# saiprasadbarke/robustmvd

Measured on AMD Instinct MI355X. Metric: depth-maps/sec at 768x1152x4srcx256planes; warp+aggregate HBM GB/s vs roofline, higher is better.
Workload: dtype f32; 1 GPU; mvsnet (Path B) forward 768x1152, 4 source views, 256 planes, batch 1 per step (BASELINE.json configs[2]); the regulariser's two layers with 32 input channels (conv0, conv4): every fp32 operand as two range-scaled fp16 terms on fp16 MFMA, fp32 accumulation (at least as close to a float64 convolution as the fp32 matrix instruction over 1e-42..1e30: tests/test_hip_f16.py), the other nine layers and ; parallelism=1 independent replica(s), frames round-robin, no collectives

## Files before the change

### robustmvd_amd/csrc/conv3d.hip

```cpp
#include "mvd_common.h"
#include <stdlib.h>

namespace mvd {

typedef float f32x4 __attribute__((ext_vector_type(4)));
typedef float f32x2 __attribute__((ext_vector_type(2)));
typedef unsigned int u32x4c __attribute__((ext_vector_type(4)));

constexpr int CONV_TH = 4;
constexpr int CONV_PAD = 4;

struct ConvParams {
    const float* x;
    const float* wpk;
    const float* scale;
    const float* shift;
    const float* skip;
    float* y;
    float* absmax;
    int B, Di, hi, wi;
    int Do, ho, wo;
    int Cout;
    int relu;
    int tiles_w, tiles_h;
    int per_xcd;
};

__device__ __forceinline__ int tile_index(const ConvParams& p) {
    const int bx = blockIdx.x;
    return (p.per_xcd > 0 && bx < 8 * p.per_xcd) ? (bx % 8) * p.per_xcd + bx / 8 : bx;
}
static int xcd_run(long long nblk, int bit) {
    const char* e = exp_env("MVD_K4_XCD");
    return (e && ((atoi(e) >> bit) & 1)) ? (int)(nblk / 8) : 0;
}

template <int CIN>
struct KGroup {
    static constexpr int KG = CIN >= 16 ? 16 : CIN;
    static constexpr int R = KG / 4;
    static constexpr int NKG = CIN / KG;
};

template <int CIN>
__host__ __device__ constexpr size_t packed_floats(int nt, int taps = 27) {
    return (size_t)taps * KGroup<CIN>::NKG * nt * 64 * KGroup<CIN>::R;
}
constexpr int MVD_CONV3D_S1_PAIR = 3;


template <int R>
__device__ __forceinline__ void load_frag(const float* src, float (&dst)[R]) {
    static_assert(R == 4 || R == 2, "k-groups of 16 or 8 channels");
    if constexpr (R == 4) {
        const float4 t = *reinterpret_cast<const float4*>(src);
        dst[0] = t.x; dst[1] = t.y; dst[2] = t.z; dst[3] = t.w;
    } else {
        const float2 t = *reinterpret_cast<const float2*>(src);
        dst[0] = t.x; dst[1] = t.y;
    }
}

__device__ __forceinline__ int decode_tile(const ConvParams& p, int bx, int& tw, int& th) {
    tw = bx % p.tiles_w; bx /= p.tiles_w;
    th = bx % p.tiles_h;
    return bx / p.tiles_h;
}

template <int CIN>
__global__ void pack_weights_kernel(const float* __restrict__ w, float* __restrict__ packed, int Cout, int NT,
                                    int transposed) {
    using G = KGroup<CIN>;
    const bool pair = transposed == 2;
    const bool dpair = transposed == 3;
    const size_t total = packed_floats<CIN>(NT, pair ? 36 : dpair ? 18 : 27);
    for (size_t e = (size_t)blockIdx.x * blockDim.x + threadIdx.x; e < total; e += (size_t)gridDim.x * blockDim.x) {
        size_t r = e;
        const int j = r % G::R; r /= G::R;
        const int lane = r % 64; r /= 64;
        const int nt = r % NT; r /= NT;
        const int g = r % G::NKG; r /= G::NKG;
        const int tap = (int)r;
        const int row = nt * 16 + (lane & 15);
        const int cin = g * G::KG + G::R * (lane >> 4) + j;
        float val = 0.f;
        if (pair) {
            const int phase = row >> 3, cout = row & 7;
            const int t = tap & 3, kdh = tap >> 2;
            const int kw = t - phase;
            if (kw >= 0 && kw <= 2) val = w[((size_t)cout * CIN + cin) * 27 + kdh * 3 + kw];
        } else if (dpair) {
            const int pw = row >> 3, cout = row & 7;
            const int st = tap & 1, kdh = tap >> 1;
            const int kw = st == 0 ? (pw ? 2 : 1) : (pw ? 0 : -1);
            if (kw >= 0) val = w[((size_t)cin * 8 + cout) * 27 + kdh * 3 + kw];
        } else if (row < Cout) {
            val = transposed ? w[((size_t)cin * Cout + row) * 27 + tap]
                             : w[((size_t)row * CIN + cin) * 27 + tap];
        }
        packed[e] = val;
    }
}

template <int MODE, int MT>
struct TileGeom {
    static constexpr bool S2 = MODE == MVD_CONV3D_STRIDE2, DECONV = MODE == MVD_DECONV3D_STRIDE2, PAIR = MODE == MVD_CONV3D_S1_PAIR;
    static constexpr int TW = 16 * MT;
    static constexpr int SX = (S2 || PAIR) ? 2 : 1;
// ... 902 lines not shown
                    for (int m = 0; m < MT; ++m)
                        acc[cls][m] = __builtin_amdgcn_mfma_f32_16x16x4f32(af[st][g][j], bf[m][j], acc[cls][m], 0, 0, 0);
            }
        }
        if (kdh + 1 < 9) {
#pragma unroll
            for (int st = 0; st < 2; ++st)
#pragma unroll
                for (int g = 0; g < G::NKG; ++g)
#pragma unroll
                    for (int j = 0; j < G::R; ++j) af[st][g][j] = af_next[st][g][j];
        }
    }

    const int arow = r0 + wave;
    if (arow >= p.hi) return;
    constexpr unsigned OOB = 0x80000000u;
    unsigned coff[MT];
#pragma unroll
    for (int m = 0; m < MT; ++m) {
        const int gcol = c0 + m * 16 + vox;
        coff[m] = gcol < p.wi ? (unsigned)(((size_t)2 * gcol * 8 + q * 4) * 4) : OOB;
    }
    const int row_bytes = p.wo * 8 * 4;
    float4 sk[4][MT];
    __amdgpu_buffer_rsrc_t yrs[4];
#pragma unroll
    for (int c = 0; c < 4; ++c) {
        const int pd = c >> 1, ph = c & 1;
        const size_t row_base = (((size_t)b * p.Do + 2 * zd + pd) * p.ho + 2 * arow + ph) * p.wo * 8;
        yrs[c] = __builtin_amdgcn_make_buffer_rsrc(p.y + row_base, 0, row_bytes, 0x00020000);
        const __amdgpu_buffer_rsrc_t srs = __builtin_amdgcn_make_buffer_rsrc(
            const_cast<float*>(p.skip ? p.skip + row_base : p.y), 0, p.skip ? row_bytes : 0, 0x00020000);
#pragma unroll
        for (int m = 0; m < MT; ++m) {
            const u32x4c t = __builtin_amdgcn_raw_buffer_load_b128(srs, coff[m], 0, 0);
            sk[c][m] = make_float4(__uint_as_float(t[0]), __uint_as_float(t[1]), __uint_as_float(t[2]), __uint_as_float(t[3]));
        }
    }
#pragma unroll
    for (int c = 0; c < 4; ++c)
#pragma unroll
        for (int m = 0; m < MT; ++m) {
            float r[4];
#pragma unroll
            for (int k = 0; k < 4; ++k) {
                r[k] = fmaf(acc[c][m][k], esc[k], esh[k]);
                if (p.relu) r[k] = fmaxf(r[k], 0.f);
            }
            __builtin_amdgcn_raw_buffer_store_b128(u32x4c{__float_as_uint(r[0] + sk[c][m].x), __float_as_uint(r[1] + sk[c][m].y),
                                                          __float_as_uint(r[2] + sk[c][m].z), __float_as_uint(r[3] + sk[c][m].w)},
                                                   yrs[c], coff[m], 0, 0);
        }
}

template <int CIN, int MT>
static int launch_deconv_pair(const ConvParams& p0, hipStream_t st) {
    ConvParams p = p0;
    constexpr size_t lds = (size_t)2 * (CONV_TH + 1) * (16 * MT + 1) * (CIN + CONV_PAD) * sizeof(float);
    static_assert(lds <= 160 * 1024, "slab exceeds LDS");
    p.tiles_h = (p.hi + CONV_TH - 1) / CONV_TH;
    p.tiles_w = (p.wi + 16 * MT - 1) / (16 * MT);
    const long long nblk = (long long)p.tiles_w * p.tiles_h * p.Di * p.B;
    p.per_xcd = xcd_run(nblk, 1);
    return launch_tiles(deconv3d_pair_kernel<CIN, MT>, nblk, 256, lds, "deconv3d_pair", p, st);
}

template <int CIN, int NT, int MT>
static int launch_deconv_all(const ConvParams& p0, hipStream_t st) {
    ConvParams p = p0;
    constexpr size_t lds = (size_t)2 * (CONV_TH + 1) * (16 * MT + 1) * (CIN + CONV_PAD) * sizeof(float);
    static_assert(lds <= 160 * 1024, "slab exceeds LDS");
    p.tiles_h = (p.hi + CONV_TH - 1) / CONV_TH;
    p.tiles_w = (p.wi + 16 * MT - 1) / (16 * MT);
    const long long nblk = (long long)p.tiles_w * p.tiles_h * p.Di * p.B;
    return launch_tiles(deconv3d_all_kernel<CIN, NT, MT>, nblk, 256, lds, "deconv3d_all", p, st);
}

constexpr int C8_DZ = 16;
constexpr int C8_TW = 62;
__global__ void __launch_bounds__(256, 4) conv3d_c8_to_1_kernel(ConvParams p) {
    constexpr int CIN = 8, TW = C8_TW, ROWS = CONV_TH + 2, COLS = TW + 2, PSTR = CIN, SLAB = ROWS * COLS * PSTR;
    static_assert(COLS == 64, "one slab column per lane");
    constexpr int NEL = ROWS * COLS * 2, NPF = (NEL + 255) / 256, DZ = C8_DZ;
    __shared__ __attribute__((aligned(16))) float ring[3 * SLAB + 4];
    const int tid = threadIdx.x, lane = tid & 63, wave = tid >> 6;
    int tw, th;
    const int bx = decode_tile(p, tile_index(p), tw, th);
    const int nzc = (p.Do + DZ - 1) / DZ;
    const int zc = bx % nzc;
    const int b = bx / nzc;
    const int r0 = th * CONV_TH, c0 = tw * TW;
    const int z0 = zc * DZ, z1 = min(z0 + DZ, p.Do);

    int loff[NPF], goff[NPF];
#pragma unroll
    for (int i = 0; i < NPF; ++i) {
        const int e = tid + 256 * i;
        const int row = e / (COLS * 2), rem = e - row * (COLS * 2);
        const int col = rem >> 1, c4 = rem & 1;
        const int gr = r0 - 1 + row, gc = c0 - 1 + col;
        constexpr int DUMMY = (3 * SLAB) / 4;
        loff[i] = e < NEL ? ((row * COLS + col) * PSTR) / 4 + c4 : DUMMY;
        goff[i] = (e < NEL && gr >= 0 && gr < p.hi && gc >= 0 && gc < p.wi) ? (gr * p.wi + gc) * 2 + c4 : -1;
    }
    const size_t plane_f4 = (size_t)p.hi * p.wi * 2;
    const float4* __restrict__ xb = reinterpret_cast<const float4*>(p.x) + (size_t)b * p.Di * plane_f4;
    float4* __restrict__ ring4 = reinterpret_cast<float4*>(ring);
    float4 pf[NPF];
    bool pf_ok = false;
    auto load_plane = [&](int plane) {
        const bool ok = plane >= 0 && plane < p.Di;
        const float4* __restrict__ xp = xb + (size_t)(ok ? plane : 0) * plane_f4;
        pf_ok = ok;
#pragma unroll
        for (int i = 0; i < NPF; ++i) pf[i] = xp[max(goff[i], 0)];
    };
    auto store_plane = [&](int slot) {
        constexpr int DUMMY = (3 * SLAB) / 4;
#pragma unroll
        for (int i = 0; i < NPF; ++i)
            ring4[loff[i] == DUMMY ? DUMMY : slot * (SLAB / 4) + loff[i]] =
                (pf_ok && goff[i] >= 0) ? pf[i] : make_float4(0.f, 0.f, 0.f, 0.f);
    };
    load_plane(z0 - 1);
    store_plane((z0 + 2) % 3);
    load_plane(z0);
    store_plane(z0 % 3);
    load_plane(z0 + 1);

    const int orow = r0 + wave, ocol = c0 + lane - 1;
    const bool live = lane >= 1 && lane <= TW && orow < p.ho && ocol < p.wo;
    const float sc = p.scale[0], sh = p.shift[0];
    for (int z = z0; z < z1; ++z) {
        __syncthreads();
        store_plane((z + 1) % 3);
        __syncthreads();
        if (z + 1 < z1) load_plane(z + 2);
        f32x2 qa[3], qb[3];
#pragma unroll
        for (int kw = 0; kw < 3; ++kw) { qa[kw] = f32x2{0.f, 0.f}; qb[kw] = f32x2{0.f, 0.f}; }
#pragma unroll
        for (int kd = 0; kd < 3; ++kd) {
            const float* __restrict__ slab = ring + ((z + kd + 2) % 3) * SLAB;
#pragma unroll
            for (int kh = 0; kh < 3; ++kh) {
                const f32x4* sp = reinterpret_cast<const f32x4*>(slab + ((wave + kh) * COLS + lane) * PSTR);
                const f32x4 a = sp[0], c = sp[1];
#pragma unroll
                for (int kw = 0; kw < 3; ++kw) {
                    typedef const __attribute__((address_space(4))) f32x4* cf4;
                    const cf4 wp = (cf4)(unsigned long long)(p.wpk + ((kd * 3 + kh) * 3 + kw) * 8);
                    const f32x4 w0 = wp[0], w1 = wp[1];
                    qa[kw] = __builtin_elementwise_fma(a.xy, w0.xy, qa[kw]);
                    qb[kw] = __builtin_elementwise_fma(a.zw, w0.zw, qb[kw]);
                    qa[kw] = __builtin_elementwise_fma(c.xy, w1.xy, qa[kw]);
                    qb[kw] = __builtin_elementwise_fma(c.zw, w1.zw, qb[kw]);
                }
            }
        }
        float q[3];
#pragma unroll
        for (int kw = 0; kw < 3; ++kw) q[kw] = (qa[kw].x + qa[kw].y) + (qb[kw].x + qb[kw].y);
        const float acc = (__shfl_up(q[0], 1) + q[1]) + __shfl_down(q[2], 1);
        if (live) {
            const size_t o = (((size_t)b * p.Do + z) * p.ho + orow) * p.wo + ocol;
            float val = fmaf(acc, sc, sh);
            if (p.relu) val = fmaxf(val, 0.f);
            if (p.skip) val += p.skip[o];
            p.y[o] = val;
        }
    }
}

__global__ void pack_c8_to_1_kernel(const float* __restrict__ w, float* __restrict__ packed) {
    const int e = blockIdx.x * blockDim.x + threadIdx.x;
    if (e < 216) packed[e] = w[(e % 8) * 27 + e / 8];
}

template <int CIN, int NT, int MT, int MODE>
static int launch_conv(const ConvParams& p0, hipStream_t st) {
    ConvParams p = p0;
    using T = TileGeom<MODE, MT>;
    constexpr size_t lds = (size_t)T::ROWS * T::COLS * (CIN + CONV_PAD) * sizeof(float) + 16;
    static_assert(lds <= 160 * 1024, "slab exceeds LDS");
    const int gh = T::DECONV ? p.hi : p.ho;
    const int gw = T::DECONV ? p.wi : T::PAIR ? (p.wo + 1) / 2 : p.wo;
    p.tiles_h = (gh + CONV_TH - 1) / CONV_TH;
    p.tiles_w = (gw + T::TW - 1) / T::TW;
    const long long nz = T::DECONV ? (long long)p.Di * 4 : p.Do;
    const long long nblk = (long long)p.tiles_w * p.tiles_h * nz * p.B;
    return launch_tiles(conv3d_kernel<CIN, NT, MT, MODE>, nblk, 256, lds, "conv3d", p, st);
}

static int launch_c8_to_1(const ConvParams& p0, hipStream_t st) {
    ConvParams p = p0;
    p.tiles_h = (p.ho + CONV_TH - 1) / CONV_TH;
    p.tiles_w = (p.wo + C8_TW - 1) / C8_TW;
    const long long nblk = (long long)p.tiles_w * p.tiles_h * ((p.Do + C8_DZ - 1) / C8_DZ) * p.B;
    p.per_xcd = xcd_run(nblk, 0);
    return launch_tiles(conv3d_c8_to_1_kernel, nblk, 256, 0, "conv3d_c8_to_1", p, st);
}

static int best_mt(int cols, int lo, int hi) {
    int best = hi, waste = 1 << 30;
    for (int mt = hi; mt >= lo; --mt) {
        const int tw = 16 * mt, pad = (cols + tw - 1) / tw * tw - cols;
        if (pad < waste) { waste = pad; best = mt; }
    }
    return best;
}

template <int CIN, int NT, int MTMAX, int MODE>
static int launch_conv_best(const ConvParams& p, hipStream_t st) {
    const int gw = MODE == MVD_DECONV3D_STRIDE2 ? p.wi : p.wo;
    if constexpr (MTMAX >= 4) {
        if (best_mt(gw, 3, 4) == 3) return launch_conv<CIN, NT, 3, MODE>(p, st);
    } else if constexpr (MTMAX == 2) {
        if (best_mt(gw, 1, 2) == 1) return launch_conv<CIN, NT, 1, MODE>(p, st);
    }
    return launch_conv<CIN, NT, MTMAX, MODE>(p, st);
}

template <int CIN, int NT, int MTMAX>
static int launch_march_best(const ConvParams& p, hipStream_t st) {
    if constexpr (MTMAX >= 4) {
#ifdef MVD_EXPERIMENTS
        if (const char* e = exp_env("MVD_K4_MARCH_MT")) {
            if (atoi(e) == 1) return launch_march<CIN, NT, 1, false>(p, st);
            if (atoi(e) == 2) return launch_march<CIN, NT, 2, false>(p, st);
        }
#endif
        if (best_mt(p.wo, 3, 4) == 3) return launch_march<CIN, NT, 3, false>(p, st);
    }
    return launch_march<CIN, NT, MTMAX, false>(p, st);
}

template <int CIN, int MODE>
static int dispatch_cout(const ConvParams& p, hipStream_t st) {
    constexpr int MT = MODE == MVD_CONV3D_STRIDE2 ? (CIN >= 32 ? 2 : 4) : 4;
    if constexpr (MODE == MVD_CONV3D_STRIDE1) {
        const bool old = exp_env("MVD_K4_NOMARCH") != nullptr;
        if (p.Cout == 8) {
            if constexpr (CIN == 32)
                if (!old && !p.skip && !exp_env("MVD_K4_NOKSPLIT")) {
                    int rc = -1;
#ifdef MVD_EXPERIMENTS
                    const char* dz = exp_env("MVD_K4_CONV0_DZ");
                    if (dz && atoi(dz) == 32) rc = launch_conv0_ksplit<32>(p, st);
                    else if (dz && atoi(dz) == 64) rc = launch_conv0_ksplit<64>(p, st);
                    else
#endif
                        rc = launch_conv0_ksplit<16>(p, st);
                    if (rc >= 0) return rc;
                }
            if constexpr (CIN <= 32)
                if (!old) {
                    const int rc = launch_march<CIN, 1, (CIN >= 32 ? 1 : 2), true>(p, st);
                    if (rc >= 0) return rc;
                }
            return launch_conv<CIN, 1, (CIN >= 64 ? 1 : 2), MVD_CONV3D_S1_PAIR>(p, st);
        }
        if (p.Cout == 1 && CIN == 8) return launch_c8_to_1(p, st);
        if constexpr (CIN >= 16)
            if (!old) {
                constexpr int MM = CIN == 16 ? 4 : CIN == 32 ? 2 : 1;
                int rc = -1;
                switch ((p.Cout + 15) / 16) {
                    case 1: rc = launch_march_best<CIN, 1, MM>(p, st); break;
                    case 2: rc = launch_march_best<CIN, 2, MM>(p, st); break;
                    case 4: rc = launch_march_best<CIN, 4, MM>(p, st); break;
                }
                if (rc >= 0) return rc;
            }
    }
    const int nt = (p.Cout + 15) / 16;
    if constexpr (MODE == MVD_DECONV3D_STRIDE2) {
        if (p.Cout == 8) {
            if constexpr (CIN >= 64) {
                return launch_deconv_pair<CIN, 2>(p, st);
            } else {
                switch (best_mt(p.wi, 2, 4)) {
// ... 127 lines not shown
```

### robustmvd_amd/csrc/conv3d_split.hip

```cpp
#include "mvd_common.h"

#ifndef SPLIT_KO
#define SPLIT_KO 0
#endif
#ifndef SPLIT_DEPTH
#define SPLIT_DEPTH 4
#endif

namespace mvd {

typedef _Float16 h16x8 __attribute__((ext_vector_type(8)));
typedef float sf32x4 __attribute__((ext_vector_type(4)));
typedef unsigned int su32x4 __attribute__((ext_vector_type(4)));
typedef unsigned int su32x2 __attribute__((ext_vector_type(2)));
typedef _Float16 h16x2 __attribute__((ext_vector_type(2)));

constexpr int S_TH = 4, S_TW = 32, S_ROWS = S_TH + 2;
template <int CIN>
struct SplitGeom {
    static constexpr int CH8 = CIN / 8;
    static constexpr int VB = CIN * 2;
    static constexpr int KWG = CIN == 32 ? 3 : 2;
    static constexpr int NT = 9 * KWG;
    static constexpr int COLS = CIN == 32 ? S_TW + 2 : S_TW + 3;
    static constexpr int HALF_BYTES = S_ROWS * COLS * VB;
    static constexpr int PLANE_BYTES = 2 * HALF_BYTES;
    static constexpr int ITEMS = S_ROWS * COLS * CH8;
    static constexpr int NLOAD = (ITEMS + 255) / 256;
    static constexpr int NF = 4 * KWG * 2;
    static_assert(NF - 8 == 4 * NLOAD, "pass B interleaves 8 epilogue groups and 4 staging groups per item");
};

__global__ void conv0_split_wscale_kernel(const float* __restrict__ w, float* __restrict__ wscale, int cin) {
    __shared__ float red[256];
    const int c = blockIdx.x;
    float m = 0.f;
    for (int e = threadIdx.x; e < cin * 27; e += 256) {
        const float v = fabsf(w[(size_t)c * cin * 27 + e]);
        m = (v <= 3.4e38f && v > m) ? v : m;
    }
    red[threadIdx.x] = m;
    __syncthreads();
    for (int o = 128; o > 0; o >>= 1) {
        if (threadIdx.x < o) red[threadIdx.x] = fmaxf(red[threadIdx.x], red[threadIdx.x + o]);
        __syncthreads();
    }
    if (threadIdx.x == 0) {
        const int ex = (int)((__float_as_uint(red[0]) >> 23) & 0xffu) - 127;
        const int k = red[0] > 0.f ? max(-100, min(100, ex - 10)) : 0;
        wscale[c] = ldexpf(1.0f, k);
    }
}

template <int CIN>
__global__ void pack_conv0_split_kernel(const float* __restrict__ w, const float* __restrict__ wscale, _Float16* __restrict__ packed, int ncb) {
    using G = SplitGeom<CIN>;
    const int e = blockIdx.x * 256 + threadIdx.x;
    if (e >= ncb * G::NT * 64 * 8) return;
    const int j = e & 7, lane = (e >> 3) & 63, t = (e >> 9) % G::NT, cb = (e >> 9) / G::NT;
    const int col = lane & 15, k = 8 * (lane >> 4) + j, cout = cb * 8 + (col & 7);
    int tap, cin;
    if constexpr (CIN == 32) { tap = t; cin = k; }
    else { const int kw = 2 * (t % 2) + k / 16; tap = kw < 3 ? (t / 2) * 3 + kw : -1; cin = k % 16; }
    const float v = tap >= 0 ? w[((size_t)cout * CIN + cin) * 27 + tap] / wscale[cout] : 0.0f;
    const _Float16 hi = (_Float16)v;
    const _Float16 lo = (_Float16)((v - (float)hi) * 2048.0f);
    packed[e] = col < 8 ? hi : lo;
}

struct SplitParams {
    const float* x;
    const char* wpk;
    const float* scale;
    const float* shift;
    const float* absmax;
    float* y;
    float* yamax;
    int B, D, h, w, relu;
    int cout, ncb;
    int tiles_x, tiles_y, dgroups, td, tiles_per_xcd;
};

__device__ __forceinline__ unsigned pack_h2(_Float16 a, _Float16 b) {
    const h16x2 v = {a, b};
    return __builtin_bit_cast(unsigned, v);
}

template <int CIN, bool YAMAX = false>
__global__ void __launch_bounds__(256, 2) conv0_split_kernel(SplitParams p) {
    using G = SplitGeom<CIN>;
    constexpr int S_COLS = G::COLS, S_HALF_BYTES = G::HALF_BYTES, S_PLANE_BYTES = G::PLANE_BYTES, S_ITEMS = G::ITEMS, S_NLOAD = G::NLOAD;
    constexpr int KWG = G::KWG, NT = G::NT;
    extern __shared__ __attribute__((aligned(16))) char ring[];
    const int tid = threadIdx.x, lane = tid & 63, wv = tid >> 6;
    const int D = p.D, h = p.h, w = p.w;

    const int xcd = blockIdx.x & 7;
    int j = blockIdx.x >> 3;
    const int cb = j % p.ncb; j /= p.ncb;
    const int t_in = j % p.tiles_per_xcd; j /= p.tiles_per_xcd;
    const int dg = j % p.dgroups;
    const int b = j / p.dgroups;
    const int tile = xcd * p.tiles_per_xcd + t_in;
    if (tile >= p.tiles_x * p.tiles_y) return;
    const int ty = tile / p.tiles_x, tx = tile - ty * p.tiles_x;
    const int x0 = tx * S_TW, y0 = ty * S_TH;
    const int dz0 = dg * p.td, dz1 = min(dz0 + p.td, D);

    h16x8 wf[NT];
#pragma unroll
    for (int t = 0; t < NT; ++t) wf[t] = *reinterpret_cast<const h16x8*>(p.wpk + (((size_t)cb * NT + t) * 64 + lane) * 16);

    constexpr unsigned OOB = 0x80000000u;
    unsigned gob[S_NLOAD];
    int loff[S_NLOAD];
#pragma unroll
    for (int k = 0; k < S_NLOAD; ++k) {
        const int e = tid + 256 * k;
        const int vox = e / G::CH8, ch = e % G::CH8;
        const int r = vox / S_COLS, c = vox - r * S_COLS;
        const int gy = y0 - 1 + r, gx = x0 - 1 + c;
        const bool in = e < S_ITEMS && c < S_TW + 2 && gy >= 0 && gy < h && gx >= 0 && gx < w;
        gob[k] = in ? (unsigned)(((gy * w + gx) * CIN + ch * 8) * 4) : OOB;
        if constexpr (CIN == 32) loff[k] = e < S_ITEMS ? (vox * 64 + ((ch ^ ((c >> 1) & 3)) * 16)) : -1;
        else loff[k] = e < S_ITEMS ? e * 16 : -1;
    }
    const size_t plane_f = (size_t)h * w * CIN;
    const float* xb = p.x + (size_t)b * D * plane_f;
    su32x4 pre[S_NLOAD][2];
    auto fetch = [&](int d) {
        const bool din = d >= 0 && d < D && d <= dz1;
        const __amdgpu_buffer_rsrc_t rs = __builtin_amdgcn_make_buffer_rsrc(
            const_cast<float*>(xb + (din ? (size_t)d * plane_f : 0)), 0, din ? (int)(plane_f * 4) : 0, 0x00020000);
#pragma unroll
        for (int k = 0; k < S_NLOAD; ++k) {
            pre[k][0] = __builtin_amdgcn_raw_buffer_load_b128(rs, gob[k], 0, 0);
            pre[k][1] = __builtin_amdgcn_raw_buffer_load_b128(rs, gob[k] + 16u, 0, 0);
        }
    };
    char* const dump = ring + 2 * S_PLANE_BYTES + tid * 16;
    float k2048 = 2048.0f, xs, xs_inv;
    {
        const unsigned mb = __builtin_amdgcn_readfirstlane((int)__float_as_uint(*p.absmax));
        const int ex = (int)((mb >> 23) & 0xffu) - 127;
        const int e = max(-125, min(125, ex - 14));
        xs = __uint_as_float((unsigned)(127 - e) << 23);
        xs_inv = __uint_as_float((unsigned)(127 + e) << 23);
    }
    auto split2 = [k2048, xs](float a0, float a1, unsigned& hi, unsigned& lo) {
        unsigned hp, lp;
        float t0, t1;
        asm("v_fma_mixlo_f16 %0, %1, %2, 0 op_sel:[0,0,0] op_sel_hi:[0,0,0]" : "=v"(hp) : "v"(a0), "s"(xs));
        asm("v_fma_mixhi_f16 %0, %1, %2, 0 op_sel:[0,0,0] op_sel_hi:[0,0,0]" : "+v"(hp) : "v"(a1), "s"(xs));
        asm("v_fma_mix_f32 %0, %1, %2, -%3 op_sel:[0,0,0] op_sel_hi:[0,0,1]" : "=v"(t0) : "v"(a0), "s"(xs), "v"(hp));
        asm("v_fma_mix_f32 %0, %1, %2, -%3 op_sel:[0,0,1] op_sel_hi:[0,0,1]" : "=v"(t1) : "v"(a1), "s"(xs), "v"(hp));
        asm("v_fma_mixlo_f16 %0, %1, %2, 0 op_sel:[0,0,0] op_sel_hi:[0,0,0]" : "=v"(lp) : "v"(t0), "s"(k2048));
        asm("v_fma_mixhi_f16 %0, %1, %2, 0 op_sel:[0,0,0] op_sel_hi:[0,0,0]" : "+v"(lp) : "v"(t1), "s"(k2048));
        hi = hp;
        lo = lp;
    };
    auto stash = [&](int d) {
        char* slot = ring + (d & 1) * S_PLANE_BYTES;
#pragma unroll
        for (int k = 0; k < S_NLOAD; ++k) {
            su32x4 hv, lv;
#pragma unroll
            for (int q = 0; q < 4; ++q) {
                const sf32x4 v = __builtin_bit_cast(sf32x4, pre[k][q >> 1]);
                unsigned hi, lo;
                split2(v[(q & 1) * 2], v[(q & 1) * 2 + 1], hi, lo);
                hv[q] = hi; lv[q] = lo;
            }
            char* dst = loff[k] >= 0 ? slot + loff[k] : dump;
            *reinterpret_cast<su32x4*>(dst) = hv;
            *reinterpret_cast<su32x4*>(loff[k] >= 0 ? dst + S_HALF_BYTES : dst) = lv;
        }
    };

    const int col = lane & 15;
    float esc_ = p.scale[cb * 8 + (col & 7)], esh_ = p.shift[cb * 8 + (col & 7)];
    float eun_ = reinterpret_cast<const float*>(p.wpk + (size_t)p.ncb * NT * 64 * 16)[cb * 8 + (col & 7)] * xs_inv;
    const float floor_ = p.relu ? 0.f : -__builtin_inff();
    const int xh = wv & 1, rp = wv >> 1;

    int fragk[KWG];
#pragma unroll
    for (int kw = 0; kw < KWG; ++kw) {
        if constexpr (CIN == 32) {
            const int c = 16 * xh + (lane & 15) + kw;
            fragk[kw] = (2 * rp * S_COLS + c) * 64 + (((lane >> 4) ^ ((c >> 1) & 3)) * 16);
        } else {
            const int c = 16 * xh + (lane & 15) + 2 * kw;
            fragk[kw] = (2 * rp * S_COLS + c) * 32 + (lane >> 4) * 16;
        }
    }

    sf32x4 acc[3][2][2];
#pragma unroll
    for (int s = 0; s < 3; ++s)
#pragma unroll
        for (int r = 0; r < 2; ++r) { acc[s][r][0] = sf32x4{0, 0, 0, 0}; acc[s][r][1] = sf32x4{0, 0, 0, 0}; }

    unsigned yoff[2];
#pragma unroll
    for (int row = 0; row < 2; ++row) {
        const int oy = y0 + 2 * rp + row;
        yoff[row] = (col < 8 && oy < h) ? (unsigned)((((size_t)oy * w + x0 + 16 * xh + 4 * (lane >> 4)) * p.cout + cb * 8 + col) * 4) : OOB;
    }
    const int oxb = x0 + 16 * xh + 4 * (lane >> 4);
    const size_t yplane_f = (size_t)h * w * p.cout;
    const unsigned vox_b = (unsigned)p.cout * 4u;

    fetch(dz0 - 1);
    asm volatile("" : "+v"(esc_), "+v"(esh_), "+v"(eun_));
    stash(dz0 - 1);
    fetch(dz0);

    [[maybe_unused]] float amax_ = 0.f;
    for (int z = dz0 - 1; z <= dz1; ++z) {
        if (!(SPLIT_KO & 8)) __syncthreads();
        const char* slot = ring + (z & 1) * S_PLANE_BYTES;
        char* wslot = ring + ((z + 1) & 1) * S_PLANE_BYTES;
        const int din = z + 2, dout = z - 1;
        const bool in_ok = din >= 0 && din < D && din <= dz1, out_ok = dout >= dz0 && dout < dz1;
        const __amdgpu_buffer_rsrc_t rs_in = __builtin_amdgcn_make_buffer_rsrc(
            const_cast<float*>(xb + (in_ok ? (size_t)din * plane_f : 0)), 0, in_ok ? (int)(plane_f * 4) : 0, 0x00020000);
        const __amdgpu_buffer_rsrc_t rs_out = __builtin_amdgcn_make_buffer_rsrc(
            p.y + ((size_t)b * D + (out_ok ? dout : 0)) * yplane_f, 0, out_ok ? (int)(yplane_f * 4) : 0, 0x00020000);
        int ox = oxb;
        asm volatile("" : "+v"(ox));

        constexpr int NF = G::NF, NR = 2 * NF, DEPTH = SPLIT_DEPTH;
        h16x8 fr[DEPTH];
        auto rr_of = [](int ro) { return ro == 0 ? 1 : ro == 1 ? 2 : ro == 2 ? 0 : 3; };
        auto frag = [&](int i) {
            const int g = i % NF, term = g & 1, kw = (g >> 1) % KWG, rr = rr_of(g / (2 * KWG));
            if (SPLIT_KO & 32) return wf[i % NT];
            return *reinterpret_cast<const h16x8*>(slot + term * S_HALF_BYTES + fragk[kw] + rr * S_COLS * G::VB);
        };
#pragma unroll
        for (int i = 0; i < DEPTH; ++i) fr[i] = frag(i);
#pragma unroll
        for (int g = 0; g < NF; ++g) {
            const int term = g & 1, kw = (g >> 1) % KWG, rr = rr_of(g / (2 * KWG));
            const h16x8 f = fr[g % DEPTH];
#pragma unroll
            for (int row = 0; row < 2; ++row) {
                const int kh = rr - row;
                if (kh < 0 || kh > 2) continue;
                if (SPLIT_KO & 16) acc[0][row][term][0] += f[0] * wf[(6 + kh) * KWG + kw][0];
                else acc[0][row][term] = __builtin_amdgcn_mfma_f32_16x16x32_f16(f, wf[(6 + kh) * KWG + kw], acc[0][row][term], 0, 0, 0);
            }
            fr[g % DEPTH] = frag(g + DEPTH);
            __builtin_amdgcn_sched_barrier(0);
        }
        float hl = __shfl_down(acc[0][0][0][0], 8, 16);
        unsigned hq0 = 0, lq0 = 0;
#pragma unroll
        for (int g = 0; g < NF; ++g) {
            const int term = g & 1, kw = (g >> 1) % KWG, rr = rr_of(g / (2 * KWG));
            const h16x8 f = fr[(NF + g) % DEPTH];
#pragma unroll
            for (int row = 0; row < 2; ++row) {
                const int kh = rr - row;
                if (kh < 0 || kh > 2) continue;
#pragma unroll
                for (int s = 1; s < 3; ++s)
                    if (SPLIT_KO & 16) acc[s][row][term][0] += f[0] * wf[((2 - s) * 3 + kh) * KWG + kw][0];
                    else acc[s][row][term] = __builtin_amdgcn_mfma_f32_16x16x32_f16(f, wf[((2 - s) * 3 + kh) * KWG + kw], acc[s][row][term], 0, 0, 0);
            }
            if (NF + g + DEPTH < NR) fr[(NF + g) % DEPTH] = frag(NF + g + DEPTH);
            if (g < 8) {
                const int row = g >> 2, i = g & 3;
                const float cur = hl;
                if (g + 1 < 8) hl = __shfl_down(acc[0][(g + 1) >> 2][0][(g + 1) & 3], 8, 16);
                float r = __builtin_fmaf(cur + acc[0][row][1][i], 1.0f / 2048.0f, acc[0][row][0][i]);
                r = fmaxf(__builtin_fmaf(r * eun_, esc_, esh_), floor_);
                if constexpr (YAMAX)
                    if (out_ok && yoff[row] != OOB && ox + i < w) amax_ = fmaxf(amax_, finite_abs_or_zero(r));
                if (!(SPLIT_KO & 2) || r == 12345.678f)
                    __builtin_amdgcn_raw_buffer_store_b32(__float_as_uint(r), rs_out, ox + i < w ? yoff[row] + vox_b * i : OOB, 0, 0);
            } else if (!(SPLIT_KO & 4)) {
                const int k = (g - 8) >> 2, q = (g - 8) & 3;
                const sf32x4 v = __builtin_bit_cast(sf32x4, pre[k][q >> 1]);
                unsigned hq1, lq1;
                split2(v[(q & 1) * 2], v[(q & 1) * 2 + 1], hq1, lq1);
                if (q & 1) {
                    char* dst = (loff[k] >= 0 ? wslot + loff[k] : dump) + 8 * (q >> 1);
                    *reinterpret_cast<su32x2*>(dst) = su32x2{hq0, hq1};
                    *reinterpret_cast<su32x2*>(loff[k] >= 0 ? dst + S_HALF_BYTES : dst) = su32x2{lq0, lq1};
                } else {
                    hq0 = hq1; lq0 = lq1;
                }
                if (q == 3 && !(SPLIT_KO & 1)) {
                    pre[k][0] = __builtin_amdgcn_raw_buffer_load_b128(rs_in, gob[k], 0, 0);
                    pre[k][1] = __builtin_amdgcn_raw_buffer_load_b128(rs_in, gob[k] + 16u, 0, 0);
                }
            }
            __builtin_amdgcn_sched_barrier(0);
        }
#pragma unroll
        for (int r = 0; r < 2; ++r)
#pragma unroll
            for (int t = 0; t < 2; ++t) {
                acc[0][r][t] = acc[1][r][t];
                acc[1][r][t] = acc[2][r][t];
                acc[2][r][t] = sf32x4{0, 0, 0, 0};
            }
    }
    if constexpr (YAMAX) {
        for (int o = 32; o > 0; o >>= 1) amax_ = fmaxf(amax_, __shfl_xor(amax_, o));
        __syncthreads();
        float* wm = reinterpret_cast<float*>(ring);
        if (lane == 0) wm[wv] = amax_;
        __syncthreads();
        if (tid == 0) {
            amax_ = fmaxf(fmaxf(wm[0], wm[1]), fmaxf(wm[2], wm[3]));
            raise_absmax(p.yamax, amax_);
        }
    }
}

}

static bool split_shape_ok(int Cin, int Cout) { return (Cin == 32 || Cin == 16) && Cout >= 8 && Cout <= 64 && Cout % 8 == 0; }
static size_t split_frag_bytes(int Cin, int Cout) { return (size_t)(Cout / 8) * (Cin == 32 ? 27 : 18) * 64 * 16; }

template <int CIN, bool YAMAX>
static int launch_split_v(const mvd::SplitParams& p, long long nblk, hipStream_t st) {
    const size_t lds = 2 * (size_t)mvd::SplitGeom<CIN>::PLANE_BYTES + 256 * 16;
    (void)hipFuncSetAttribute((const void*)mvd::conv0_split_kernel<CIN, YAMAX>, hipFuncAttributeMaxDynamicSharedMemorySize, (int)lds);
    hipLaunchKernelGGL((mvd::conv0_split_kernel<CIN, YAMAX>), dim3((unsigned)nblk), dim3(256), lds, st, p);
    return mvd::launch_status("conv3d_split");
}
template <int CIN>
static int launch_split(const mvd::SplitParams& p, long long nblk, hipStream_t st) {
    return p.yamax ? launch_split_v<CIN, true>(p, nblk, st) : launch_split_v<CIN, false>(p, nblk, st);
}

extern "C" {

size_t mvd_conv3d_split_packed_weight_bytes(int Cin, int Cout) {
    return split_shape_ok(Cin, Cout) ? split_frag_bytes(Cin, Cout) + (size_t)Cout * sizeof(float) : 0;
}

int mvd_pack_conv3d_weights_split(const float* w, int Cin, int Cout, void* packed, mvd_stream_t stream) {
    MVD_REQUIRE(w && packed, "pack_conv3d_weights_split: NULL argument");
    MVD_REQUIRE(split_shape_ok(Cin, Cout), "pack_conv3d_weights_split: 16 or 32 input channels and 8, 16, ... 64 output channels are built (got %d -> %d)", Cin, Cout);
    const int ncb = Cout / 8;
    float* wscale = reinterpret_cast<float*>(static_cast<char*>(packed) + split_frag_bytes(Cin, Cout));
    hipLaunchKernelGGL(mvd::conv0_split_wscale_kernel, dim3(Cout), dim3(256), 0, (hipStream_t)stream, w, wscale, Cin);
    const unsigned nb = (unsigned)((split_frag_bytes(Cin, Cout) / 2 + 255) / 256);
    if (Cin == 32) hipLaunchKernelGGL(mvd::pack_conv0_split_kernel<32>, dim3(nb), dim3(256), 0, (hipStream_t)stream, w, wscale, (_Float16*)packed, ncb);
    else hipLaunchKernelGGL(mvd::pack_conv0_split_kernel<16>, dim3(nb), dim3(256), 0, (hipStream_t)stream, w, wscale, (_Float16*)packed, ncb);
    return mvd::launch_status("pack_conv3d_weights_split");
}

static int conv3d_split_entry(const float* x, const float* x_absmax, const void* packed_w, const float* scale, const float* shift, float* y,
                              float* y_absmax, int B, int D, int h, int w, int Cin, int Cout, int relu, mvd_stream_t stream);

int mvd_conv3d_bn_relu_f32_split(const float* x, const float* x_absmax, const void* packed_w, const float* scale, const float* shift,
                                 float* y, int B, int D, int h, int w, int Cin, int Cout, int relu, mvd_stream_t stream) {
    return conv3d_split_entry(x, x_absmax, packed_w, scale, shift, y, nullptr, B, D, h, w, Cin, Cout, relu, stream);
}

int mvd_conv3d_bn_relu_absmax_f32_split(const float* x, const float* x_absmax, const void* packed_w, const float* scale, const float* shift,
                                        float* y, float* y_absmax, int B, int D, int h, int w, int Cin, int Cout, int relu,
                                        mvd_stream_t stream) {
    MVD_REQUIRE(y_absmax, "conv3d_split_absmax: NULL argument");
    return conv3d_split_entry(x, x_absmax, packed_w, scale, shift, y, y_absmax, B, D, h, w, Cin, Cout, relu, stream);
}

static int conv3d_split_entry(const float* x, const float* x_absmax, const void* packed_w, const float* scale, const float* shift, float* y,
                              float* y_absmax, int B, int D, int h, int w, int Cin, int Cout, int relu, mvd_stream_t stream) {
    MVD_REQUIRE(x && x_absmax && packed_w && scale && shift && y, "conv3d_split: NULL argument");
    MVD_REQUIRE(split_shape_ok(Cin, Cout), "conv3d_split: 16 or 32 input channels and 8, 16, ... 64 output channels are built (got %d -> %d)", Cin, Cout);
    MVD_REQUIRE(B > 0 && D > 0 && h > 0 && w > 0, "conv3d_split: non-positive dimension");
    MVD_REQUIRE((long long)h * w * Cin * 4 < 0x7fffffffLL && (long long)h * w * Cout * 4 < 0x7fffffffLL,
                "conv3d_split: one plane exceeds the 31-bit byte-offset range");
    mvd::SplitParams p{};
    p.x = x; p.absmax = x_absmax; p.wpk = (const char*)packed_w; p.scale = scale; p.shift = shift; p.y = y; p.yamax = y_absmax;
    if (y_absmax && hipMemsetAsync(y_absmax, 0, sizeof(float), (hipStream_t)stream) != hipSuccess) return mvd::launch_status("conv3d_split: memset");
    p.B = B; p.D = D; p.h = h; p.w = w; p.relu = relu;
    p.cout = Cout; p.ncb = Cout / 8;
    p.tiles_x = (w + mvd::S_TW - 1) / mvd::S_TW;
    p.tiles_y = (h + mvd::S_TH - 1) / mvd::S_TH;
    const long long tiles = (long long)p.tiles_x * p.tiles_y;
    p.tiles_per_xcd = (int)((tiles + 7) / 8);
    int td = 32;
    while (td > 8 && tiles * B * p.ncb * ((D + td - 1) / td) < 2048) td /= 2;
    p.td = td;
    p.dgroups = (D + td - 1) / td;
    const long long nblk = 8LL * p.ncb * p.tiles_per_xcd * p.dgroups * B;
    MVD_REQUIRE(nblk <= 0x7fffffffLL, "conv3d_split: %lld workgroups exceed the grid limit", nblk);
    return Cin == 32 ? launch_split<32>(p, nblk, (hipStream_t)stream) : launch_split<16>(p, nblk, (hipStream_t)stream);
}
}
```

Baseline: 333.3 depth-maps/sec.

## Cut the c8-to-1 conv ring to two plane slots and template split conv tile height

The c8->1 3D conv kernel now keeps a two-slot LDS ring instead of three. Each input plane is loaded once and scattered into three rotating per-depth accumulator sets, with the depth chunk taken from a runtime parameter. This shrinks LDS per block to raise occupancy, at the cost of more accumulator registers and extra conditional steps. The split fp16 conv gets a templated tile height (4 or 8 rows), selectable only through an environment variable; the old three-slot kernel is kept behind an experiments flag.

```diff
diff --git a/robustmvd_amd/csrc/conv3d.hip b/robustmvd_amd/csrc/conv3d.hip
--- a/robustmvd_amd/csrc/conv3d.hip
+++ b/robustmvd_amd/csrc/conv3d.hip
@@ -1,5 +1,6 @@
 #include "mvd_common.h"
 #include <stdlib.h>
+#include <type_traits>
 
 namespace mvd {
 
@@ -24,6 +25,7 @@
     int relu;
     int tiles_w, tiles_h;
     int per_xcd;
+    int dz;
 };
 
 __device__ __forceinline__ int tile_index(const ConvParams& p) {
@@ -1092,7 +1094,123 @@
 __global__ void __launch_bounds__(256, 4) conv3d_c8_to_1_kernel(ConvParams p) {
     constexpr int CIN = 8, TW = C8_TW, ROWS = CONV_TH + 2, COLS = TW + 2, PSTR = CIN, SLAB = ROWS * COLS * PSTR;
     static_assert(COLS == 64, "one slab column per lane");
-    constexpr int NEL = ROWS * COLS * 2, NPF = (NEL + 255) / 256, DZ = C8_DZ;
+    constexpr int NEL = ROWS * COLS * 2, NPF = (NEL + 255) / 256, DUMMY = (2 * SLAB) / 4;
+    __shared__ __attribute__((aligned(16))) float ring[2 * SLAB + 4];
+    const int tid = threadIdx.x, lane = tid & 63, wave = tid >> 6;
+    int tw, th;
+    const int bx = decode_tile(p, tile_index(p), tw, th);
+    const int nzc = (p.Do + p.dz - 1) / p.dz;
+    const int zc = bx % nzc;
+    const int b = bx / nzc;
+    const int r0 = th * CONV_TH, c0 = tw * TW;
+    const int z0 = zc * p.dz, z1 = min(z0 + p.dz, p.Do);
+
+    int loff[NPF], goff[NPF];
+#pragma unroll
+    for (int i = 0; i < NPF; ++i) {
+        const int e = tid + 256 * i;
+        const int row = e / (COLS * 2), rem = e - row * (COLS * 2);
+        const int col = rem >> 1, c4 = rem & 1;
+        const int gr = r0 - 1 + row, gc = c0 - 1 + col;
+        loff[i] = e < NEL ? ((row * COLS + col) * PSTR) / 4 + c4 : DUMMY;
+        goff[i] = (e < NEL && gr >= 0 && gr < p.hi && gc >= 0 && gc < p.wi) ? (gr * p.wi + gc) * 2 + c4 : -1;
+    }
+    const size_t plane_f4 = (size_t)p.hi * p.wi * 2;
+    const float4* __restrict__ xb = reinterpret_cast<const float4*>(p.x) + (size_t)b * p.Di * plane_f4;
+    float4* __restrict__ ring4 = reinterpret_cast<float4*>(ring);
+    float4 pf[NPF];
+    bool pf_ok = false;
+    auto load_plane = [&](int plane) {
+        const bool ok = plane >= 0 && plane < p.Di;
+        const float4* __restrict__ xp = xb + (size_t)(ok ? plane : 0) * plane_f4;
+        pf_ok = ok;
+#pragma unroll
+        for (int i = 0; i < NPF; ++i) pf[i] = xp[max(goff[i], 0)];
+    };
+    auto store_plane = [&](int plane) {
+        const int slot = (plane + 2) & 1;
+#pragma unroll
+        for (int i = 0; i < NPF; ++i)
+            ring4[loff[i] == DUMMY ? DUMMY : slot * (SLAB / 4) + loff[i]] =
+                (pf_ok && goff[i] >= 0) ? pf[i] : make_float4(0.f, 0.f, 0.f, 0.f);
+    };
+    load_plane(z0 - 1);
+    store_plane(z0 - 1);
+    load_plane(z0);
+
+    const int orow = r0 + wave, ocol = c0 + lane - 1;
+    const bool live = lane >= 1 && lane <= TW && orow < p.ho && ocol < p.wo;
+    const float sc = p.scale[0], sh = p.shift[0];
+    f32x2 qa[3][3], qb[3][3];
+#pragma unroll
+    for (int s = 0; s < 3; ++s)
+#pragma unroll
+        for (int kw = 0; kw < 3; ++kw) { qa[s][kw] = f32x2{0.f, 0.f}; qb[s][kw] = f32x2{0.f, 0.f}; }
+
+    auto step = [&](auto ph, int z) {
+        constexpr int PH = decltype(ph)::value;
+        __syncthreads();
+        if (z < z1) store_plane(z + 1);
+        if (z + 1 < z1) load_plane(z + 2);
+        const float* wl = p.wpk;
+        asm volatile("" : "+s"(wl));
+        const float* __restrict__ slab = ring + ((z + 2) & 1) * SLAB;
+        f32x4 a[3], c[3];
+#pragma unroll
+        for (int kh = 0; kh < 3; ++kh) {
+            const f32x4* sp = reinterpret_cast<const f32x4*>(slab + ((wave + kh) * COLS + lane) * PSTR);
+            a[kh] = sp[0];
+            c[kh] = sp[1];
+        }
+        auto taps = [&](auto kdc) {
+            constexpr int kd = decltype(kdc)::value, S = (PH + 2 - kd) % 3;
+#pragma unroll
+            for (int kh = 0; kh < 3; ++kh)
+#pragma unroll
+                for (int kw = 0; kw < 3; ++kw) {
+                    typedef const __attribute__((address_space(4))) f32x4* cf4;
+                    const cf4 wp = (cf4)(unsigned long long)(wl + ((kd * 3 + kh) * 3 + kw) * 8);
+                    const f32x4 w0 = wp[0], w1 = wp[1];
+                    qa[S][kw] = __builtin_elementwise_fma(a[kh].xy, w0.xy, qa[S][kw]);
+                    qb[S][kw] = __builtin_elementwise_fma(a[kh].zw, w0.zw, qb[S][kw]);
+                    qa[S][kw] = __builtin_elementwise_fma(c[kh].xy, w1.xy, qa[S][kw]);
+                    qb[S][kw] = __builtin_elementwise_fma(c[kh].zw, w1.zw, qb[S][kw]);
+                }
+        };
+        if (z + 1 < z1) taps(std::integral_constant<int, 0>{});
+        if (z >= z0 && z < z1) taps(std::integral_constant<int, 1>{});
+        if (z > z0) {
+            taps(std::integral_constant<int, 2>{});
+            float q[3];
+#pragma unroll
+            for (int kw = 0; kw < 3; ++kw) q[kw] = (qa[PH][kw].x + qa[PH][kw].y) + (qb[PH][kw].x + qb[PH][kw].y);
+            const float acc = (__shfl_up(q[0], 1) + q[1]) + __shfl_down(q[2], 1);
+            if (live) {
+                const size_t o = (((size_t)b * p.Do + (z - 1)) * p.ho + orow) * p.wo + ocol;
+                float val = fmaf(acc, sc, sh);
+                if (p.relu) val = fmaxf(val, 0.f);
+                if (p.skip) val += p.skip[o];
+                p.y[o] = val;
+            }
+        }
+#pragma unroll
+        for (int kw = 0; kw < 3; ++kw) { qa[PH][kw] = f32x2{0.f, 0.f}; qb[PH][kw] = f32x2{0.f, 0.f}; }
+    };
+    for (int z = z0 - 1; z <= z1; z += 3) {
+        step(std::integral_constant<int, 0>{}, z);
+        if (z + 1 > z1) break;
+        step(std::integral_constant<int, 1>{}, z + 1);
+        if (z + 2 > z1) break;
+        step(std::integral_constant<int, 2>{}, z + 2);
+    }
+}
+
+#ifdef MVD_EXPERIMENTS
+constexpr int C8_RING3_DZ = 16;
+__global__ void __launch_bounds__(256, 4) conv3d_c8_to_1_ring3_kernel(ConvParams p) {
+    constexpr int CIN = 8, TW = C8_TW, ROWS = CONV_TH + 2, COLS = TW + 2, PSTR = CIN, SLAB = ROWS * COLS * PSTR;
+    static_assert(COLS == 64, "one slab column per lane");
+    constexpr int NEL = ROWS * COLS * 2, NPF = (NEL + 255) / 256, DZ = C8_RING3_DZ;
     __shared__ __attribute__((aligned(16))) float ring[3 * SLAB + 4];
     const int tid = threadIdx.x, lane = tid & 63, wave = tid >> 6;
     int tw, th;
@@ -1182,6 +1300,8 @@
         }
     }
 }
+
+#endif
 
 __global__ void pack_c8_to_1_kernel(const float* __restrict__ w, float* __restrict__ packed) {
     const int e = blockIdx.x * blockDim.x + threadIdx.x;
@@ -1207,7 +1327,16 @@
     ConvParams p = p0;
     p.tiles_h = (p.ho + CONV_TH - 1) / CONV_TH;
     p.tiles_w = (p.wo + C8_TW - 1) / C8_TW;
-    const long long nblk = (long long)p.tiles_w * p.tiles_h * ((p.Do + C8_DZ - 1) / C8_DZ) * p.B;
+    p.dz = C8_DZ;
+#ifdef MVD_EXPERIMENTS
+    if (exp_env("MVD_K4_PROB_RING3")) {
+        const long long nold = (long long)p.tiles_w * p.tiles_h * ((p.Do + C8_RING3_DZ - 1) / C8_RING3_DZ) * p.B;
+        p.per_xcd = xcd_run(nold, 0);
+        return launch_tiles(conv3d_c8_to_1_ring3_kernel, nold, 256, 0, "conv3d_c8_to_1_ring3", p, st);
+    }
+    if (const char* e = exp_env("MVD_K4_PROB_DZ")) p.dz = max(1, atoi(e));
+#endif
+    const long long nblk = (long long)p.tiles_w * p.tiles_h * ((p.Do + p.dz - 1) / p.dz) * p.B;
     p.per_xcd = xcd_run(nblk, 0);
     return launch_tiles(conv3d_c8_to_1_kernel, nblk, 256, 0, "conv3d_c8_to_1", p, st);
 }
diff --git a/robustmvd_amd/csrc/conv3d_split.hip b/robustmvd_amd/csrc/conv3d_split.hip
--- a/robustmvd_amd/csrc/conv3d_split.hip
+++ b/robustmvd_amd/csrc/conv3d_split.hip
@@ -15,20 +15,24 @@
 typedef unsigned int su32x2 __attribute__((ext_vector_type(2)));
 typedef _Float16 h16x2 __attribute__((ext_vector_type(2)));
 
-constexpr int S_TH = 4, S_TW = 32, S_ROWS = S_TH + 2;
-template <int CIN>
+constexpr int S_TW = 32;
+template <int CIN, int TH = 4>
 struct SplitGeom {
+    static_assert(TH == 4 || TH == 8, "two output rows per wave, 4 or 8 waves");
+    static constexpr int ROWS = TH + 2;
+    static constexpr int NTHR = 64 * TH;
     static constexpr int CH8 = CIN / 8;
     static constexpr int VB = CIN * 2;
     static constexpr int KWG = CIN == 32 ? 3 : 2;
     static constexpr int NT = 9 * KWG;
     static constexpr int COLS = CIN == 32 ? S_TW + 2 : S_TW + 3;
-    static constexpr int HALF_BYTES = S_ROWS * COLS * VB;
+    static constexpr int HALF_BYTES = ROWS * COLS * VB;
     static constexpr int PLANE_BYTES = 2 * HALF_BYTES;
-    static constexpr int ITEMS = S_ROWS * COLS * CH8;
-    static constexpr int NLOAD = (ITEMS + 255) / 256;
+    static constexpr int ITEMS = ROWS * COLS * CH8;
+    static constexpr int NLOAD = (ITEMS + NTHR - 1) / NTHR;
+    static constexpr size_t LDS_BYTES = 2 * (size_t)PLANE_BYTES + NTHR * 16;
     static constexpr int NF = 4 * KWG * 2;
-    static_assert(NF - 8 == 4 * NLOAD, "pass B interleaves 8 epilogue groups and 4 staging groups per item");
+    static_assert(NF - 8 >= 4 * NLOAD, "pass B interleaves 8 epilogue groups and 4 staging groups per item");
 };
 
 __global__ void conv0_split_wscale_kernel(const float* __restrict__ w, float* __restrict__ wscale, int cin) {
@@ -86,10 +90,10 @@
     return __builtin_bit_cast(unsigned, v);
 }
 
-template <int CIN, bool YAMAX = false>
-__global__ void __launch_bounds__(256, 2) conv0_split_kernel(SplitParams p) {
-    using G = SplitGeom<CIN>;
-    constexpr int S_COLS = G::COLS, S_HALF_BYTES = G::HALF_BYTES, S_PLANE_BYTES = G::PLANE_BYTES, S_ITEMS = G::ITEMS, S_NLOAD = G::NLOAD;
+template <int CIN, int TH, bool YAMAX = false>
+__global__ void __launch_bounds__(64 * TH, 2) conv0_split_kernel(SplitParams p) {
+    using G = SplitGeom<CIN, TH>;
+    constexpr int NTHR = G::NTHR, S_COLS = G::COLS, S_HALF_BYTES = G::HALF_BYTES, S_PLANE_BYTES = G::PLANE_BYTES, S_ITEMS = G::ITEMS, S_NLOAD = G::NLOAD;
     constexpr int KWG = G::KWG, NT = G::NT;
     extern __shared__ __attribute__((aligned(16))) char ring[];
     const int tid = threadIdx.x, lane = tid & 63, wv = tid >> 6;
@@ -104,7 +108,7 @@
     const int tile = xcd * p.tiles_per_xcd + t_in;
     if (tile >= p.tiles_x * p.tiles_y) return;
     const int ty = tile / p.tiles_x, tx = tile - ty * p.tiles_x;
-    const int x0 = tx * S_TW, y0 = ty * S_TH;
+    const int x0 = tx * S_TW, y0 = ty * TH;
     const int dz0 = dg * p.td, dz1 = min(dz0 + p.td, D);
 
     h16x8 wf[NT];
@@ -116,7 +120,7 @@
     int loff[S_NLOAD];
 #pragma unroll
     for (int k = 0; k < S_NLOAD; ++k) {
-        const int e = tid + 256 * k;
+        const int e = tid + NTHR * k;
         const int vox = e / G::CH8, ch = e % G::CH8;
         const int r = vox / S_COLS, c = vox - r * S_COLS;
         const int gy = y0 - 1 + r, gx = x0 - 1 + c;
@@ -280,8 +284,8 @@
                     if (out_ok && yoff[row] != OOB && ox + i < w) amax_ = fmaxf(amax_, finite_abs_or_zero(r));
                 if (!(SPLIT_KO & 2) || r == 12345.678f)
                     __builtin_amdgcn_raw_buffer_store_b32(__float_as_uint(r), rs_out, ox + i < w ? yoff[row] + vox_b * i : OOB, 0, 0);
-            } else if (!(SPLIT_KO & 4)) {
-                const int k = (g - 8) >> 2, q = (g - 8) & 3;
+            } else if (g - 8 < 4 * S_NLOAD && !(SPLIT_KO & 4)) {
+                const int k = min((g - 8) >> 2, S_NLOAD - 1), q = (g - 8) & 3;
                 const sf32x4 v = __builtin_bit_cast(sf32x4, pre[k][q >> 1]);
                 unsigned hq1, lq1;
                 split2(v[(q & 1) * 2], v[(q & 1) * 2 + 1], hq1, lq1);
@@ -315,7 +319,8 @@
         if (lane == 0) wm[wv] = amax_;
         __syncthreads();
         if (tid == 0) {
-            amax_ = fmaxf(fmaxf(wm[0], wm[1]), fmaxf(wm[2], wm[3]));
+            amax_ = wm[0];
+            for (int i = 1; i < TH; ++i) amax_ = fmaxf(amax_, wm[i]);
             raise_absmax(p.yamax, amax_);
         }
     }
@@ -326,16 +331,29 @@
 static bool split_shape_ok(int Cin, int Cout) { return (Cin == 32 || Cin == 16) && Cout >= 8 && Cout <= 64 && Cout % 8 == 0; }
 static size_t split_frag_bytes(int Cin, int Cout) { return (size_t)(Cout / 8) * (Cin == 32 ? 27 : 18) * 64 * 16; }
 
-template <int CIN, bool YAMAX>
+template <int CIN, int TH, bool YAMAX>
 static int launch_split_v(const mvd::SplitParams& p, long long nblk, hipStream_t st) {
-    const size_t lds = 2 * (size_t)mvd::SplitGeom<CIN>::PLANE_BYTES + 256 * 16;
-    (void)hipFuncSetAttribute((const void*)mvd::conv0_split_kernel<CIN, YAMAX>, hipFuncAttributeMaxDynamicSharedMemorySize, (int)lds);
-    hipLaunchKernelGGL((mvd::conv0_split_kernel<CIN, YAMAX>), dim3((unsigned)nblk), dim3(256), lds, st, p);
+    using G = mvd::SplitGeom<CIN, TH>;
+    static_assert(G::LDS_BYTES <= 160 * 1024, "the two plane slots exceed the LDS");
+    (void)hipFuncSetAttribute((const void*)mvd::conv0_split_kernel<CIN, TH, YAMAX>, hipFuncAttributeMaxDynamicSharedMemorySize, (int)G::LDS_BYTES);
+    hipLaunchKernelGGL((mvd::conv0_split_kernel<CIN, TH, YAMAX>), dim3((unsigned)nblk), dim3(G::NTHR), G::LDS_BYTES, st, p);
     return mvd::launch_status("conv3d_split");
 }
-template <int CIN>
+template <int CIN, int TH>
 static int launch_split(const mvd::SplitParams& p, long long nblk, hipStream_t st) {
-    return p.yamax ? launch_split_v<CIN, true>(p, nblk, st) : launch_split_v<CIN, false>(p, nblk, st);
+    return p.yamax ? launch_split_v<CIN, TH, true>(p, nblk, st) : launch_split_v<CIN, TH, false>(p, nblk, st);
+}
+
+static long long split_grid(mvd::SplitParams& p, int th) {
+    p.tiles_x = (p.w + mvd::S_TW - 1) / mvd::S_TW;
+    p.tiles_y = (p.h + th - 1) / th;
+    const long long tiles = (long long)p.tiles_x * p.tiles_y;
+    p.tiles_per_xcd = (int)((tiles + 7) / 8);
+    int td = 32;
+    while (td > 8 && tiles * p.B * p.ncb * ((p.D + td - 1) / td) * th < 2048 * 4) td /= 2;
+    p.td = td;
+    p.dgroups = (p.D + td - 1) / td;
+    return 8LL * p.ncb * p.tiles_per_xcd * p.dgroups * p.B;
 }
 
 extern "C" {
@@ -383,16 +401,13 @@
     if (y_absmax && hipMemsetAsync(y_absmax, 0, sizeof(float), (hipStream_t)stream) != hipSuccess) return mvd::launch_status("conv3d_split: memset");
     p.B = B; p.D = D; p.h = h; p.w = w; p.relu = relu;
     p.cout = Cout; p.ncb = Cout / 8;
-    p.tiles_x = (w + mvd::S_TW - 1) / mvd::S_TW;
-    p.tiles_y = (h + mvd::S_TH - 1) / mvd::S_TH;
-    const long long tiles = (long long)p.tiles_x * p.tiles_y;
-    p.tiles_per_xcd = (int)((tiles + 7) / 8);
-    int td = 32;
-    while (td > 8 && tiles * B * p.ncb * ((D + td - 1) / td) < 2048) td /= 2;
-    p.td = td;
-    p.dgroups = (D + td - 1) / td;
-    const long long nblk = 8LL * p.ncb * p.tiles_per_xcd * p.dgroups * B;
+    int th = 4;
+    if (const char* e = mvd::exp_env("MVD_K4_SPLIT_TH")) {
+        if (Cin == 32) th = atoi(e) == 8 ? 8 : 4;
+    }
+    const long long nblk = split_grid(p, th);
     MVD_REQUIRE(nblk <= 0x7fffffffLL, "conv3d_split: %lld workgroups exceed the grid limit", nblk);
-    return Cin == 32 ? launch_split<32>(p, nblk, (hipStream_t)stream) : launch_split<16>(p, nblk, (hipStream_t)stream);
-}
-}
+    if (Cin == 16) return launch_split<16, 4>(p, nblk, (hipStream_t)stream);
+    return th == 8 ? launch_split<32, 8>(p, nblk, (hipStream_t)stream) : launch_split<32, 4>(p, nblk, (hipStream_t)stream);
+}
+}
```

Result: no change. 333.3 depth-maps/sec (-0.0%).
